# ViTAE-Transformer/LeMeViT

Measured on AMD Instinct MI355X. Metric: images/sec LeMeViT-Base 224^2 bf16 fwd+bwd, higher is better.
Workload: dtype bf16; 1 GPU; lemevit_base 224x224 bf16-autocast train step (fwd+bwd+AdamW), batch 128/GPU, drop_path 0.1, random-init weights; global_batch=128, parallelism=dp1, launch=eager, weight-gradient GEMMs on a side stream

## Files before the change

### include/lemevit_hip.h

```cpp
#ifndef LEMEVIT_HIP_H
#define LEMEVIT_HIP_H

#include <stddef.h>
#include <stdint.h>

#ifdef __cplusplus
extern "C" {
#endif

#define LMV_ABI_VERSION 14

enum { LMV_F32 = 0, LMV_BF16 = 1, LMV_U8 = 2  };
enum {
  LMV_OK = 0,
  LMV_ERR_SHAPE = -1,
  LMV_ERR_DTYPE = -2,
  LMV_ERR_WORKSPACE = -3,
  LMV_ERR_LAUNCH = -4
};

int lmv_abi_version(void);
const char* lmv_last_error(void);
int lmv_config_set(const char* key, int value);
int lmv_config_get(const char* key, int* value);
// ... 149 lines not shown
int lmv_row_scale(const void* x, const float* scale, void* y, int64_t rows, int C, int rows_per_sample, int dtype, void* stream);
typedef struct lmv_row_scale_segment {
  const void* x; const float* scale; void* y;
  int64_t rows; int rows_per_sample;
} lmv_row_scale_segment;
int lmv_row_scale_multi(const lmv_row_scale_segment* seg, int nseg, int C, int dtype, void* stream);
#define LMV_TRANSPOSE_MAX_SEGS 48
typedef struct { const void* src; void* dst; int32_t rows, cols; } lmv_transpose_seg;
int lmv_transpose_batch(const lmv_transpose_seg* segs, int nsegs, int dtype, void* stream);
int lmv_im2col3x3s2_nhwc(const void* x, void* patches, int B, int H, int W, int C, int KP, int dtype, void* stream);
int lmv_col2im3x3s2_nhwc(const void* dpatches, void* dx, int B, int H, int W, int C, int KP, int dtype, void* stream);
int lmv_conv3x3s2_fwd(const void* x, const void* wm, const float* bias, void* y, int B, int H, int W, int Cin, int Cout, int KP, int act, int dtype, void* stream);
size_t lmv_conv3x3s2_dw_workspace_bytes(int B, int H, int W, int Cin, int Cout, int KP, int dtype);
int lmv_conv3x3s2_dw(const void* dy, const void* x, float* dwm, float* dbias, int B, int H, int W, int Cin, int Cout, int KP, void* workspace, size_t workspace_bytes, int dtype,
                     void* stream);
enum { LMV_FOLD_CI_TAP = 0, LMV_FOLD_TAP_CI = 1 };
int lmv_conv_bn_fold(const float* w, const float* b, const float* gamma, const float* beta, const float* mean, const float* var, float eps, int Co, int Cin, int KP,
                     int layout, void* wm, float* bf, float* sc, int dtype, void* stream);
int lmv_conv_bn_fold_bwd(const float* dwm, const float* dbf, const float* w, const float* b, const float* gamma, const float* mean, const float* var, float eps, int Co,
                         int Cin, int KP, int layout, float* dW, float* db, float* dgamma, float* dbeta, void* stream);
int lmv_token_mean2_fwd(const void* x, int L, const void* c, int M, int C, int B, void* out, int dtype, void* stream);
int lmv_token_mean2_bwd(const void* g, void* dx, int L, void* dc, int M, int C, int B, int dtype, void* stream);
int lmv_token_mean2_affine_fwd(const void* x, int L, const void* c, int M, int C, int B, const float* xscale, const float* xshift, void* out, int dtype,
                               void* stream);
int lmv_adamw_flat(float* param, const float* grad, float* exp_avg, float* exp_avg_sq, const float* wd_mask, void* shadow_bf16,
                   int64_t n, float lr, float beta1, float beta2, float eps, float weight_decay, int step, const int* step_dev,
                   void* stream);
typedef struct { const float* ptr; int64_t n; } lmv_norm_seg;
#define LMV_GRAD_STAT_FLOATS 8
#define LMV_NORM_CHUNK 16384
// ... 206 lines not shown
```

### lemevit_amd/_lib.py

```python
from __future__ import annotations

import ctypes as C
import os

import torch

_HERE = os.path.dirname(os.path.abspath(__file__))
LIB_PATH = os.environ.get("LMV_LIB_PATH") or os.path.join(_HERE, "csrc", "liblemevit_hip.so")

LMV_F32, LMV_BF16, LMV_U8 = 0, 1, 2
ACT_NONE, ACT_GELU, ACT_GELU_GRAD, ACT_GELU_BWD = 0, 1, 2, 3
FOLD_CI_TAP, FOLD_TAP_CI = 0, 1
ABI_VERSION = 14
BLOCK_NO_JOIN, BLOCK_FUSED, BLOCK_DATA_ONLY = 1, 2, 4
GRAD_STAT_FLOATS, NORM_CHUNK, NORM_SKIP_NONFINITE = 8, 16384, 1
ADAMW_UNIT, ADAMW_MAX_GROUPS = 8, 256
ERASE_MAX_BOXES = 4
ERASE_CONST, ERASE_RAND, ERASE_PIXEL = 0, 1, 2
EVAL_MAX_PRED, METER_MAX_K = 16, 8
DENSE_MAX_CLASSES, DENSE_STATS_HEAD = 64, 6
DENSE_LABEL_I64, DENSE_LABEL_U8 = 0, 1
DENSE_AVG_VALID, DENSE_AVG_ALL, DENSE_AVG_WEIGHT = 0, 1, 2
DENSE_SLIDE_MAX_GRID = 64
RROI_MAX_LEVELS, RROI_MAX_SAMPLE_NUM, RROI_MAX_BINS, RROI_MAX_SAMPLES, RROI_MAX_EXTENT = 5, 4, 256, 1024, 65535
# ... 150 lines not shown
    "lmv_dca_core_fwd": (_I, [_P, _P, _P, _P, _P, _P, _I, _I, _I, _I, _P, _Z, _I, _P]),
    "lmv_cast": (_I, [_P, _I, _P, _I, _L, _P]),
    "lmv_im2col3x3s2_c3": (_I, [_P, _I, _P, _I, _I, _I, _I, _L, _L, _L, _L, _P]),
    "lmv_im2col3x3s2_nchw": (_I, [_P, _I, _P, _I, _I, _I, _I, _I, _I, _L, _L, _L, _L, _P]),
    "lmv_conv3x3s2_nchw_dx": (_I, [_P, _P, _P, _I, _I, _I, _I, _I, _I, _I, _L, _L, _L, _L, _I, _P]),
    "lmv_row_scale_multi": (_I, [_P, _I, _I, _I, _P]),
    "lmv_transpose_batch": (_I, [C.POINTER(TransposeSeg), _I, _I, _P]),
    "lmv_row_scale": (_I, [_P, _P, _P, _L, _I, _I, _I, _P]),
    "lmv_im2col3x3s2_nhwc": (_I, [_P, _P, _I, _I, _I, _I, _I, _I, _P]),
    "lmv_conv3x3s2_fwd": (_I, [_P, _P, _P, _P, _I, _I, _I, _I, _I, _I, _I, _I, _P]),
    "lmv_conv3x3s2_dw_workspace_bytes": (_Z, [_I, _I, _I, _I, _I, _I, _I]),
    "lmv_conv3x3s2_dw": (_I, [_P, _P, _P, _P, _I, _I, _I, _I, _I, _I, _P, _Z, _I, _P]),
    "lmv_conv_bn_fold": (_I, [_P, _P, _P, _P, _P, _P, _F, _I, _I, _I, _I, _P, _P, _P, _I, _P]),
    "lmv_conv_bn_fold_bwd": (_I, [_P, _P, _P, _P, _P, _P, _P, _F, _I, _I, _I, _I, _P, _P, _P, _P, _P]),
    "lmv_col2im3x3s2_nhwc": (_I, [_P, _P, _I, _I, _I, _I, _I, _I, _P]),
    "lmv_token_mean2_fwd": (_I, [_P, _I, _P, _I, _I, _I, _P, _I, _P]),
    "lmv_token_mean2_affine_fwd": (_I, [_P, _I, _P, _I, _I, _I, _P, _P, _P, _I, _P]),
    "lmv_token_mean2_bwd": (_I, [_P, _P, _I, _P, _I, _I, _I, _I, _P]),
    "lmv_adamw_flat": (_I, [_P, _P, _P, _P, _P, _P, _L, _F, _F, _F, _F, _F, _I, _P, _P]),
    "lmv_grad_norm_workspace_bytes": (_Z, [C.POINTER(NormSeg), _I]),
    "lmv_grad_norm": (_I, [C.POINTER(NormSeg), _I, _F, _I, _P, _P, _P, _Z, _P]),
    "lmv_adamw_flat_clip": (_I, [_P, _P, _P, _P, _P, _P, _L, _F, _F, _F, _F, _F, _I, _P, _P, _F, _P]),
    "lmv_adamw_flat_groups": (_I, [_P, _P, _P, _P, _P, _L, _P, _P, _I, _F, _F, _F, _I, _P, _P, _F, _P]),
    "lmv_ema_flat": (_I, [_P, _P, _L, _F, _P]),
    "lmv_mix_images": (_I, [_P, _I, _L, _L, _L, _L, _P, _I, _I, _I, _I, _I, _P, _P, _P, _P, _P]),
    "lmv_soft_ce": (_I, [_P, _I, _L, _I, _I, _P, _P, _F, _P, _I, _L, _P, _P, _P, _P]),
    "lmv_augment_images": (_I, [_P, _I, _L, _L, _L, _L, _P, _I, _I, _I, _I, _I, _P, _P, _P, _P, _I, _P, _P, _P, _P]),
    "lmv_eval_logits": (_I, [_P, _I, _L, _I, _I, _P, _I, _P, _P, _P, _I, _P]),
    "lmv_meter_add": (_I, [_P, _P, _P, _I, C.POINTER(C.c_int32), _I, _P, _L, _P]),
    "lmv_dense_loss_workspace_bytes": (_Z, [_I, _I, _L]),
# ... 96 lines not shown
```

### lemevit_amd/csrc/gemm.hip

```cpp
#include <stdlib.h>
#include <atomic>
#include <utility>
#include "common.h"

#include "gemm_tiles.h"

namespace {

template <typename T, bool ATR, bool BTR, bool SPLITK, int BK, bool DMA, typename CF, int MINW = 1, int NST = 2, bool LNP = false, bool CONV = false>
__global__ __launch_bounds__(CF::NTHR, MINW) void gemm_kernel(const GemmArgs g) {
  static_assert(!LNP || (!ATR && !BTR && !SPLITK), "the LayerNorm-folded epilogue belongs to the forward contraction");
  static_assert(!CONV || (DMA && ((!ATR && !BTR && !SPLITK) || (ATR && BTR && SPLITK))), "the implicit-GEMM convolution: the LDS-DMA forward and weight-gradient kernels");
  using RS = typename std::conditional<LNP, RowStat<CF::WM>, NoStat>::type;
  RS rstat;
  if constexpr (LNP) rstat.clear();
#ifdef LMV_GEMM_TIMING
  const bool tstamp = g.dbg && (threadIdx.x == 0) && (blockIdx.x == 0 || blockIdx.x == gridDim.x / 2);
  unsigned long long* const tdbg = g.dbg + (blockIdx.x == 0 ? 0 : 256);
  int tstn = 0;
#define GSTAMP() do { if (tstamp && tstn < 250) tdbg[tstn++] = __builtin_amdgcn_s_memtime(); } while (0)
#else
#define GSTAMP() do { } while (0)
#endif
  GSTAMP();
  constexpr int PANEL_BYTES = PANEL * BK * (int)sizeof(T);
  constexpr int BUF_BYTES = (CF::PA + CF::PB) * PANEL_BYTES;
  constexpr int WM = CF::WM;
// ... 15 lines not shown
    if (split >= g.nsplits || bid >= g.ntiles) return;
  } else {
    const int T_ = gridDim.x, xcd = blockIdx.x & 7, q = T_ >> 3, r = T_ & 7, len = q + (xcd < r ? 1 : 0);
    int idx = blockIdx.x >> 3;
    const int chunk = idx & ~127;
    if (chunk + 128 <= len) idx = chunk + ((idx & 31) << 2) + ((idx >> 5) & 3);
    bid = (xcd < r ? xcd * (q + 1) : r * (q + 1) + (xcd - r) * q) + idx;
  }
  const bool second = g.nprob > 1 && !g.concat && bid >= g.p[1].tile_begin;
  const int pi = second ? 1 : 0;
  Problem P;
#define LMV_SEL(f) P.f = second ? g.p[1].f : g.p[0].f
  LMV_SEL(a); LMV_SEL(b); LMV_SEL(bias); LMV_SEL(res); LMV_SEL(row_scale); LMV_SEL(aux); LMV_SEL(out); LMV_SEL(out_pre); LMV_SEL(bias_grad);
  LMV_SEL(M); LMV_SEL(Kred); LMV_SEL(rps); LMV_SEL(tiles_m); LMV_SEL(tile_begin);
#undef LMV_SEL
  bid -= P.tile_begin;
  const int tm = bid / g.tiles_n, tn = bid % g.tiles_n;
  const int m0 = tm * CF::BM, n0 = tn * CF::BN;
  const int M = P.M, N = g.N;
  const int kt0 = (P.Kred + BK - 1) / BK;
  const int kt_total = kt0 + ((SPLITK && g.concat) ? (g.p[1].Kred + BK - 1) / BK : 0);
  const int kt_beg = split * g.kt_per_split;
  const int kt_end = min(kt_total, kt_beg + g.kt_per_split);
  if (kt_beg >= kt_end) return;
  const T* const a0 = reinterpret_cast<const T*>(P.a); const T* const b0 = reinterpret_cast<const T*>(P.b);
  const T* const a1 = SPLITK ? reinterpret_cast<const T*>(g.p[1].a) : a0; const T* const b1 = SPLITK ? reinterpret_cast<const T*>(g.p[1].b) : b0;
  const int kred0 = P.Kred, kred1 = SPLITK ? g.p[1].Kred : P.Kred;
  auto src_of = [&](int kt, const T** a, const T** b, int* kred, int* k0) {
    const bool second = SPLITK && kt >= kt0;
    *a = second ? a1 : a0; *b = second ? b1 : b0;
// ... 7 lines not shown
#pragma unroll
    for (int j = 0; j < 4; ++j) acc[i][j] = f32x4_t{0.f, 0.f, 0.f, 0.f};
  }
  const int ra0 = wm * WM * 16, cb0 = wn * 64;
  const int pa = ra0 / PANEL, oa = ra0 % PANEL, pb = cb0 / PANEL, ob = cb0 % PANEL;
  const bool do_bsum = SPLITK && (P.bias_grad != nullptr) && tn == 0 && wn == 0;

  constexpr int REGION = NST * BUF_BYTES / CF::NW;
  constexpr bool EPI_EARLY = false;
  Epi<T, CF, SPLITK ? 4096 : REGION> epi;
  if constexpr (EPI_EARLY) epi.prefetch(P, g.act & 0xff, N, g.ldc, m0, n0, wm, wn, lane);

  int cur = 0;
  if constexpr (DMA) {
    static_assert(sizeof(T) == 2, "the direct-to-LDS path is bf16 only");
    auto issue = [&](unsigned char* buf, int kt) {
      const bf16_t *A16, *B16; int kred, k0;
      src_of(kt, &A16, &B16, &kred, &k0);
#pragma unroll
      for (int q = 0; q < CF::PA; ++q) {
        if constexpr (CONV && !SPLITK) panel_dma_conv<false, BK, CF::NW>(buf + q * PANEL_BYTES, g.cv, M, m0 + q * PANEL, k0, lane, wave);
        else panel_dma<ATR, BK, CF::NW>(buf + q * PANEL_BYTES, A16, g.lda, M, m0 + q * PANEL, k0, lane, wave);
      }
#pragma unroll
      for (int q = 0; q < CF::PB; ++q) {
        if constexpr (CONV && SPLITK) panel_dma_conv<true, BK, CF::NW>(buf + (CF::PA + q) * PANEL_BYTES, g.cv, N, n0 + q * PANEL, k0, lane, wave);
        else panel_dma<BTR, BK, CF::NW>(buf + (CF::PA + q) * PANEL_BYTES, B16, g.ldb, N, n0 + q * PANEL, k0, lane, wave);
      }
    };
    if constexpr (CF::NW >= 8 && CF::WM == 2 && NST == 2) {
      issue(smem, kt_beg);
      GSTAMP();
      __syncthreads();
      GSTAMP();
      for (int kt = kt_beg; kt < kt_end; ++kt) {
        if (kt + 1 < kt_end) issue(smem + (cur ^ 1) * BUF_BYTES, kt + 1);
        GSTAMP();
        const unsigned char* buf = smem + cur * BUF_BYTES;
        tile_mma<T, ATR, BTR, BK, SPLITK, WM, RS>(buf + pa * PANEL_BYTES, oa, buf + (CF::PA + pb) * PANEL_BYTES, ob, acc, accb, do_bsum, lane, &rstat);
        GSTAMP();
        __syncthreads();
// ... 69 lines not shown
      if (do_bsum && lane < 16) slab[(int64_t)M * g.ldc + m] = accb[ti][0];
    }
  } else {
    GSTAMP();
    if constexpr (LNP) {
      rstat.finish(P.Kred, g.ln_eps);
      epi.prefetch(P, LMV_ACT_NONE, N, g.ldc, m0, n0, wm, wn, lane);
      epi.template store<true>(smem, acc, P, g.act & 0xff, N, g.ldc, m0, n0, wm, wn, lane, wave, rstat.s, rstat.q);
    } else {
      if constexpr (!EPI_EARLY) epi.prefetch(P, g.act & 0xff, N, g.ldc, m0, n0, wm, wn, lane);
      GSTAMP();
#ifdef LMV_GEMM_TIMING
      auto est = [&]() { GSTAMP(); };
      epi.template store<false, decltype(est)>(smem, acc, P, g.act & 0xff, N, g.ldc, m0, n0, wm, wn, lane, wave, nullptr, nullptr, est);
#else
      epi.store(smem, acc, P, g.act & 0xff, N, g.ldc, m0, n0, wm, wn, lane, wave);
#endif
      GSTAMP();
    }
  }
}

template <int SL>
__global__ __launch_bounds__(256) void splitk_reduce_kernel(const float* __restrict__ ws, int nslabs, int64_t stride, float* __restrict__ out_w,
                                                           int64_t nw, float* __restrict__ out_b, int nb) {
  constexpr int EL = 256 / SL;
  __shared__ float4 red[SL > 1 ? 256 : 1];
  const int64_t n4 = (nw + (out_b ? nb : 0)) >> 2;
  const int e = threadIdx.x % EL, sl = threadIdx.x / EL;
  const int64_t i = (int64_t)blockIdx.x * EL + e;
  float4 a = make_float4(0.f, 0.f, 0.f, 0.f);
  if (i < n4) {
    const float* p = ws + i * 4;
#pragma unroll 8
    for (int s = sl; s < nslabs; s += SL) {
// ... 357 lines not shown
  return launch(&p, 1, Cout, KP, act, dtype, stream, MODE_FWD, nullptr, 0, nullptr, nullptr, &cv);
}
extern "C" size_t lmv_conv3x3s2_dw_workspace_bytes(int B, int H, int W, int Cin, int Cout, int KP, int dtype) {
  (void)Cin;
  lmv_linear_problem p{};
  p.a = p.w = p.out = (void*)16; p.rows = (int64_t)B * ((H + 1) / 2) * ((W + 1) / 2);
  return lmv_linear_dw_workspace_bytes(&p, 1, Cout, KP, dtype);
}
extern "C" int lmv_conv3x3s2_dw(const void* dy, const void* x, float* dwm, float* dbias, int B, int H, int W, int Cin, int Cout, int KP, void* workspace, size_t workspace_bytes, int dtype,
                                void* stream) {
  ConvGeo cv;
  LMV_TRY(conv_geo(&cv, x, B, H, W, Cin, Cout, KP, dtype));
  lmv_linear_problem p{};
  p.a = dy; p.w = x; p.out = dwm; p.bias_grad = dbias; p.rows = (int64_t)B * cv.HoWo;
  return launch(&p, 1, Cout, KP, LMV_ACT_NONE, dtype, stream, MODE_DW, workspace, workspace_bytes, nullptr, nullptr, &cv);
}

extern "C" int lmv_reduce_batch(const lmv_reduce_seg* segs, int nsegs, void* stream) {
  if (nsegs <= 0) return LMV_OK;
  if (!segs) LMV_FAIL(LMV_ERR_SHAPE, "reduce_batch: segs is NULL");
  hipStream_t st = (hipStream_t)stream;
  for (int s0 = 0; s0 < nsegs; s0 += LMV_REDUCE_MAX_SEGS) {
    ReduceBatch rb{};
    rb.n = nsegs - s0 < LMV_REDUCE_MAX_SEGS ? nsegs - s0 : LMV_REDUCE_MAX_SEGS;
    int blocks = 0;
    for (int i = 0; i < rb.n; ++i) {
      const lmv_reduce_seg& q = segs[s0 + i];
      if (!q.ws || !q.out_w || q.nslabs <= 0 || q.nw <= 0 || (q.nw % 4) || (q.out_b && (q.nb % 4)) || !lmv_aligned16(q.ws) || !lmv_aligned16(q.out_w) ||
          !lmv_aligned16(q.out_b) || (q.slab_stride % 4) || (q.kind != LMV_REDUCE_SLABS && q.kind != LMV_REDUCE_ROWS))
        LMV_FAIL(LMV_ERR_SHAPE, "reduce_batch: bad segment %d", s0 + i);
// ... 22 lines not shown
```

### lemevit_amd/csrc/gemm_tiles.h

```cpp
#pragma once
#include <utility>
#include "common.h"

namespace {

constexpr int PANEL = 128;

template <int NWM_, int NWN_, int WM_>
struct Cfg {
  static constexpr int NWM = NWM_, NWN = NWN_, WM = WM_;
  static constexpr int NW = NWM * NWN, NTHR = NW * 64;
  static constexpr int BM = NWM * WM * 16, BN = NWN * 64;
  static constexpr int PA = BM / PANEL, PB = BN / PANEL;
};
using C128 = Cfg<2, 2, 4>;
using C128w8 = Cfg<4, 2, 2>;

struct Problem {
  const void* a; const void* b; const float* bias; const void* res; const float* row_scale; const void* aux;
  void* out; void* out_pre; float* bias_grad;
  int M;
  int Kred;
  int rps;
  int tiles_m;
  int tile_begin;
  int pad_;
};
struct ReduceSegDev { const float* ws; float* out_w; float* out_b; int64_t stride, nw; int nslabs, nb, sl, blk0, kind, mode; };
#define LMV_CV_SHIFT 41
struct ConvGeo {
  int on, H, W, Cin, Ho, Wo, HoWo, pad_;
  unsigned long long m_cin, m_wo, m_howo;
  const void* x;
};
struct GemmArgs {
  Problem p[2];
  int nprob, N, lda, ldb, ldc, act, tiles_n, kt_per_split;
  ConvGeo cv;
  int ntiles, nsplits, concat;
  float ln_eps;
#ifdef LMV_GEMM_TIMING
  unsigned long long* dbg;
#endif
  float* ws;
  int64_t slab_stride;
  int slab_base[2];
};

template <int ROWB> __device__ __forceinline__ int swz_n(int row) { return ROWB == 64 ? ((-(row >> 2)) & 3) : ((row >> 1) & 7); }
// ... 35 lines not shown
      const int row = c / CPR, kc = c % CPR;
      off = row * ROWB + ((kc ^ swz_n<ROWB>(row)) << 4);
    } else {
      constexpr int CPR = PANEL / EPC;
      const int r = c / CPR, cc = c % CPR;
      if (sizeof(T) == 2) off = r * 256 + ((((cc >> 1) ^ swz_t(r))) << 5) + ((cc & 1) << 4);
      else off = r * 512 + (cc << 4);
    }
    *reinterpret_cast<uint4*>(s + off) = regs[i];
  }
}

typedef __attribute__((address_space(3))) void* lds_vp;
typedef const __attribute__((address_space(1))) void* glb_vp;

template <bool TR, int BK, int NW>
__device__ __forceinline__ void panel_dma(unsigned char* panel, const bf16_t* __restrict__ base, int64_t ld, int dim, int tile0, int k0,
                                          int lane, int wave) {
  constexpr int NSEG = PANEL * BK * 2 / 1024;
  static_assert(NSEG % NW == 0, "segments must divide over the waves");
#pragma unroll
  for (int i = 0; i < NSEG / NW; ++i) {
    const int sg = wave + i * NW;
    const bf16_t* src;
    if (!TR) {
      constexpr int ROWB = BK * 2, CPR = ROWB / 16, RPS = 1024 / ROWB;
      const int r = sg * RPS + lane / CPR, p = lane % CPR, kc = p ^ swz_n<ROWB>(r);
      src = base + (int64_t)min(tile0 + r, dim - 1) * ld + k0 + kc * 8;
    } else {
      const int r = sg * 4 + (lane >> 4), p16 = lane & 15, c16 = ((((p16 >> 1) ^ swz_t(r))) << 1) | (p16 & 1);
      src = base + (int64_t)(k0 + r) * ld + min(tile0 + c16 * 8, dim - 8);
    }
    __builtin_amdgcn_global_load_lds((glb_vp)src, (lds_vp)(panel + sg * 1024), 16, 0, 0);
  }
// ... 15 lines not shown
  static_assert(NSEG % NW == 0, "segments must divide over the waves");
#pragma unroll
  for (int i = 0; i < NSEG / NW; ++i) {
    const int sg = wave + i * NW;
    const bf16_t* src;
    if (!TR) {
      constexpr int ROWB = BK * 2, CPR = ROWB / 16, RPS = 1024 / ROWB;
      const int r = sg * RPS + lane / CPR, p = lane % CPR, kc = p ^ swz_n<ROWB>(r);
      src = cv_src(cv, min(tile0 + r, dim - 1), k0 + kc * 8);
    } else {
      const int r = sg * 4 + (lane >> 4), p16 = lane & 15, c16 = ((((p16 >> 1) ^ swz_t(r))) << 1) | (p16 & 1);
      src = cv_src(cv, k0 + r, min(tile0 + c16 * 8, dim - 8));
    }
    __builtin_amdgcn_global_load_lds((glb_vp)src, (lds_vp)(panel + sg * 1024), 16, 0, 0);
  }
}

template <bool TR, int BK>
__device__ __forceinline__ bf16x8_t frag_bf16(const unsigned char* s, int base, int lane, int hh) {
  if (!TR) {
    constexpr int ROWB = BK * 2;
    const int row = base + (lane & 15), kc = hh * 4 + (lane >> 4);
    return *reinterpret_cast<const bf16x8_t*>(s + row * ROWB + ((kc ^ swz_n<ROWB>(row)) << 4));
  } else {
    const int g = lane >> 4, i = lane & 15, rr = i >> 2, q = i & 3;
    const int r1 = hh * 32 + g * 8 + rr, r2 = r1 + 4, ch = base >> 4;
    typedef __attribute__((address_space(3))) bf16x4_t* lds4_t;
    bf16x4_t lo = __builtin_amdgcn_ds_read_tr16_b64_v4bf16((lds4_t)(s + r1 * 256 + ((ch ^ swz_t(r1)) << 5) + q * 8));
    bf16x4_t hi = __builtin_amdgcn_ds_read_tr16_b64_v4bf16((lds4_t)(s + r2 * 256 + ((ch ^ swz_t(r2)) << 5) + q * 8));
    return __builtin_shufflevector(lo, hi, 0, 1, 2, 3, 4, 5, 6, 7);
// ... 233 lines not shown
            const int m = min(m0 + wm * (CF::WM * 16) + p * RPP + r, P.M - 1);
            rs[p][i] = P.row_scale[m / P.rps];
          }
      }
    }
    if constexpr (HOIST_BIAS) {
#pragma unroll
      for (int tj = 0; tj < 4; ++tj) b4[tj] = bias_at(P, N, nw0 + tj * 16 + (lane >> 4) * 4);
    }
  }
  static __device__ __forceinline__ float4 bias_at(const Problem& P, int N, int n) {
    return (P.bias && n < N) ? *reinterpret_cast<const float4*>(P.bias + n) : make_float4(0.f, 0.f, 0.f, 0.f);
  }

  struct NoStamp { __device__ __forceinline__ void operator()() const {} };
  template <bool LN = false, typename ST = NoStamp>
  __device__ __forceinline__ void store(unsigned char* smem, const f32x4_t (&acc)[CF::WM][4], const Problem& P, int act, int N, int64_t ldc,
                                        int m0, int n0, int wm, int wn, int lane, int wave, const float* ln_mean = nullptr, const float* ln_rstd = nullptr,
                                        ST stamp = ST{}) const {
    float* sT = reinterpret_cast<float*>(smem + wave * REGION_BYTES);
    T* outp = reinterpret_cast<T*>(P.out);
    T* prep = reinterpret_cast<T*>(P.out_pre);
    const int nw0 = n0 + wn * 64;
#pragma unroll
    for (int p = 0; p < NPASS; ++p) {
      __builtin_amdgcn_wave_barrier();
#pragma unroll
      for (int tj = 0; tj < 4; ++tj) {
        float4 b;
        if constexpr (HOIST_BIAS) b = b4[tj]; else b = bias_at(P, N, nw0 + tj * 16 + (lane >> 4) * 4);
        float4 cs = make_float4(0.f, 0.f, 0.f, 0.f);
        if constexpr (LN) {
          const int n = nw0 + tj * 16 + (lane >> 4) * 4;
          if (n < N) cs = *reinterpret_cast<const float4*>(reinterpret_cast<const float*>(P.aux) + n);
// ... 13 lines not shown
      asm volatile("s_waitcnt lgkmcnt(0)" ::: "memory");
      __builtin_amdgcn_wave_barrier();
      stamp();
#pragma unroll
      for (int i = 0; i < NITER; ++i) {
        const int c = lane + i * 64, r = c / CPR, oc = c % CPR;
        const int m = m0 + wm * (CF::WM * 16) + p * RPP + r, n = nw0 + oc * EPC;
        if (m >= P.M || n >= N) continue;
        float v[EPC];
#pragma unroll
        for (int e = 0; e < EPC; e += 4) {
          const int c4 = (oc * EPC + e) >> 2;
          const float4 t = *reinterpret_cast<const float4*>(sT + r * 64 + ((c4 ^ (r & 7)) << 2));
          v[e] = t.x; v[e + 1] = t.y; v[e + 2] = t.z; v[e + 3] = t.w;
        }
        const int64_t o = (int64_t)m * ldc + n;
        if (prep) *reinterpret_cast<uint4*>(prep + o) = f_to_chunk<T>(v);
        if (act == LMV_ACT_GELU) {
#pragma unroll
          for (int e = 0; e < EPC; ++e) v[e] = act_gelu<T>(v[e]);
        } else if (act == LMV_ACT_GELU_GRAD) {
          float u[EPC];
          chunk_to_f<T>(pf[p][i], u);
#pragma unroll
          for (int e = 0; e < EPC; ++e) v[e] *= act_gelu_grad<T>(u[e]);
        }
        if (P.row_scale) {
          float sc;
          if constexpr (HOIST_BIAS) sc = rs[p][i]; else sc = P.row_scale[m / P.rps];
#pragma unroll
          for (int e = 0; e < EPC; ++e) v[e] *= sc;
// ... 17 lines not shown
```

### lemevit_amd/model.py

```python
from __future__ import annotations

import math
import operator
import os
import threading
import weakref
from collections import OrderedDict
from typing import Dict, List, Optional, Sequence, Tuple

import torch
import torch.nn as nn
import torch.nn.functional as F

from . import ops
from .blocks import ATTN_BWD, ATTN_FWD, BLOCK_LN_EPS, PARAM_NAMES, attention_state, block_backward, block_forward
from .ops import Prob

Tensor = torch.Tensor


def _cfg(url: str = "", **kwargs) -> dict:
    return dict(url=url, num_classes=1000, input_size=(3, 224, 224), pool_size=None, crop_pct=0.9, interpolation="bicubic",
                fixed_input_size=True, mean=(0.485, 0.456, 0.406), std=(0.229, 0.224, 0.225),
                first_conv="patch_embed.proj", classifier="head", **kwargs)
# ... 153 lines not shown
            dwm = torch.zeros(Co, KP, device=g.device, dtype=torch.float32)
            dbf = torch.zeros(Co, device=g.device, dtype=torch.float32)
            if ctx.form == "implicit":
                ops.conv3x3s2_dw(g, gathered, dwm, dbf)
            else:
                ops.linear_dw([Prob(g, gathered, dwm, bias_grad=dbf)], Co, KP)
            if folded:
                weight, bias, gamma, mean, var = sv[-5:]
                grads = list(ops.conv_bn_fold_bwd(dwm, dbf, weight, bias, gamma, mean, var, eps, layout, [bool(n) for n in need]))
            else:
                dw = dwm[:, :9 * Ci]
                dw = dw.reshape(wshape) if image else dw.reshape(Co, 3, 3, Ci).permute(0, 3, 1, 2)
                grads[:2] = (dw.to(wdt) if need[0] else None), (dbf.to(bdt) if need[1] else None)
        if need_x and image:
            dx = ops.conv3x3s2_nchw_dx(g, Wm, like=sv[0])
        elif need_x:
            dp = torch.empty(g.shape[0], KP, device=g.device, dtype=g.dtype)
            ops.linear_dx([Prob(g, Wm, dp)], Co, KP)
            dx = ops.col2im3x3s2_nhwc(dp, B, H, W, Ci).permute(0, 3, 1, 2).to(xdt)
        return (dx, grads[0], grads[1], None, grads[2], grads[3], None, None, None, None, None)


def _conv3x3s2(x: Tensor, weight: Tensor, bias: Optional[Tensor], cd: torch.dtype, bn: Optional[tuple] = None, gelu: bool = False, infer: bool = False) -> Tensor:
    if (infer or (gelu and bn is None)) and torch.is_grad_enabled() and any(t is not None and t.requires_grad for t in (x, weight, bias)):
        raise NotImplementedError("lemevit_amd: the inference fold and the fused GELU epilogue on a plain operand have no backward")
    gamma, beta, mean, var, eps = (None, None, None, None, None) if bn is None else bn
    return _Conv3x3s2Fn.apply(x, weight, bias, cd, gamma, beta, mean, var, eps, gelu, infer)


def _is_conv3x3s2p1(m: nn.Module) -> bool:
    return (isinstance(m, nn.Conv2d) and m.kernel_size == (3, 3) and m.stride == (2, 2) and m.padding == (1, 1) and m.dilation == (1, 1) and m.groups == 1
            and m.padding_mode == "zeros")


def _is_conv3x3s2(m: nn.Module, x: Tensor) -> bool:
    return (_is_conv3x3s2p1(m) and m.in_channels % 8 == 0 and m.out_channels % 8 == 0 and x.is_cuda
            and x.dtype in (torch.float32, torch.bfloat16) and m.weight.dtype in (torch.float32, torch.bfloat16))


_CONV_IMPLICIT = os.environ.get("LMV_CONV_IMPLICIT", "1") != "0"


_FROZEN_BN = os.environ.get("LMV_FROZEN_BN", "1") != "0"


def _bn_frozen(m: Optional[nn.Module]) -> bool:
    return (_FROZEN_BN and isinstance(m, nn.BatchNorm2d) and not m.training and m.track_running_stats and m.running_mean is not None and m.running_var is not None
            and m.affine and all(t.dtype == torch.float32 for t in (m.weight, m.bias, m.running_mean, m.running_var)))


def _conv_bn_pairs(m: nn.Module, bn: Optional[nn.Module], x: Tensor, cd: torch.dtype) -> bool:
    return (_bn_frozen(bn) and cd in (torch.float32, torch.bfloat16) and x.is_cuda and (_is_stem_conv1(m, x) or _is_conv3x3s2(m, x)) and m.weight.dtype == torch.float32
            and (m.bias is None or m.bias.dtype == torch.float32) and m.weight.is_contiguous() and bn.num_features == m.out_channels)


# ... 1502 lines not shown
```

### lemevit_amd/ops.py

```python
from __future__ import annotations

import ctypes as C
import math
from typing import List, Optional, Sequence, Tuple

import torch

from . import _lib
from ._lib import ACT_GELU, ACT_GELU_BWD, ACT_GELU_GRAD, ACT_NONE, FOLD_CI_TAP, FOLD_TAP_CI, AttnDesc, LinearProblem, LnSegment, check, lib

Tensor = torch.Tensor
HEAD_DIM = 32


def dtype_code(t: Tensor) -> int:
    if t.dtype == torch.float32:
        return _lib.LMV_F32
    if t.dtype == torch.bfloat16:
        return _lib.LMV_BF16
    raise TypeError(f"lemevit_amd: unsupported dtype {t.dtype} (float32 and bfloat16 only)")


_raw_stream = getattr(torch._C, "_cuda_getCurrentRawStream", None)

# ... 501 lines not shown
def conv_bn_fold_bwd(dwm: Tensor, dbf: Tensor, weight: Tensor, bias: Optional[Tensor], gamma: Tensor, mean: Tensor, var: Tensor, eps: float, layout: int,
                     want: Sequence[bool] = (True, True, True, True)):
    Co, Cin = weight.shape[0], weight.shape[1]
    if dwm.shape[0] != Co or dbf.numel() != Co:
        raise ValueError(f"conv_bn_fold_bwd: dwm {tuple(dwm.shape)} / dbf {tuple(dbf.shape)} do not match the weight {tuple(weight.shape)}")
    new = lambda w, shape: torch.empty(shape, device=weight.device, dtype=torch.float32) if w else None
    dW, db, dg, dbe = new(want[0], weight.shape), new(want[1], (Co,)), new(want[2], (Co,)), new(want[3], (Co,))
    check(lib.lmv_conv_bn_fold_bwd(_f32(dwm), _f32(dbf), _f32(weight), _f32(bias), _f32(gamma), _f32(mean), _f32(var), eps, Co, Cin, dwm.shape[1], layout,
                                   _ptr(dW), _ptr(db), _ptr(dg), _ptr(dbe), _stream()), "lmv_conv_bn_fold_bwd")
    return dW, db, dg, dbe


def col2im3x3s2_nhwc(dpatches: Tensor, B: int, H: int, W: int, C_: int) -> Tensor:
    dx = torch.empty((B, H, W, C_), device=dpatches.device, dtype=dpatches.dtype)
    check(lib.lmv_col2im3x3s2_nhwc(_ptr(dpatches), _ptr(dx), B, H, W, C_, dpatches.shape[1], dtype_code(dpatches), _stream()), "lmv_col2im3x3s2_nhwc")
    return dx


def token_mean2_fwd(x: Tensor, c: Optional[Tensor]) -> Tensor:
    B, L, C_ = x.shape
    out = torch.empty((B, C_), device=x.device, dtype=x.dtype)
    check(lib.lmv_token_mean2_fwd(_ptr(x), L, _ptr(c), 0 if c is None else c.shape[1], C_, B, _ptr(out), dtype_code(x), _stream()), "lmv_token_mean2_fwd")
    return out


def token_mean2_affine_fwd(x: Tensor, c: Optional[Tensor], xscale: Tensor, xshift: Tensor) -> Tensor:
    B, L, C_ = x.shape
    if xscale.dtype != torch.float32 or xshift.dtype != torch.float32 or xscale.numel() != C_ or xshift.numel() != C_:
        raise TypeError("token_mean2_affine_fwd: xscale / xshift must be float32 [C]")
    out = torch.empty((B, C_), device=x.device, dtype=x.dtype)
# ... 1204 lines not shown
```

Measured before the change: 4262 images/sec.

## Add implicit-GEMM data-gradient kernel for 3x3 stride-2 convs with parity-class decomposition

Replaces the conv3x3s2 input-gradient path (linear_dx into a materialized patch matrix, then col2im) with a single implicit-GEMM kernel. Output pixels are split into four stride-parity classes, each gathering only its contributing taps from dy via LDS-DMA, and results are written straight to NHWC dx. A cached transposed weight operand is built per weight version. This removes the large dpatches buffer and the col2im scatter pass, at the cost of gather address arithmetic, zero-page loads at borders, and a new code path with shape limits.

```diff
diff --git a/include/lemevit_hip.h b/include/lemevit_hip.h
--- a/include/lemevit_hip.h
+++ b/include/lemevit_hip.h
@@ -187,6 +187,9 @@
 size_t lmv_conv3x3s2_dw_workspace_bytes(int B, int H, int W, int Cin, int Cout, int KP, int dtype);
 int lmv_conv3x3s2_dw(const void* dy, const void* x, float* dwm, float* dbias, int B, int H, int W, int Cin, int Cout, int KP, void* workspace, size_t workspace_bytes, int dtype,
                      void* stream);
+int lmv_conv3x3s2_dx_supported(int B, int H, int W, int Cin, int Cout, int dtype);
+int lmv_conv3x3s2_dx_operand(const void* wm, void* wt, int Cin, int Cout, int KP, int dtype, void* stream);
+int lmv_conv3x3s2_dx(const void* dy, const void* wt, void* dx, int B, int H, int W, int Cin, int Cout, int dtype, void* stream);
 enum { LMV_FOLD_CI_TAP = 0, LMV_FOLD_TAP_CI = 1 };
 int lmv_conv_bn_fold(const float* w, const float* b, const float* gamma, const float* beta, const float* mean, const float* var, float eps, int Co, int Cin, int KP,
                      int layout, void* wm, float* bf, float* sc, int dtype, void* stream);
diff --git a/lemevit_amd/_lib.py b/lemevit_amd/_lib.py
--- a/lemevit_amd/_lib.py
+++ b/lemevit_amd/_lib.py
@@ -188,6 +188,9 @@
     "lmv_conv_bn_fold": (_I, [_P, _P, _P, _P, _P, _P, _F, _I, _I, _I, _I, _P, _P, _P, _I, _P]),
     "lmv_conv_bn_fold_bwd": (_I, [_P, _P, _P, _P, _P, _P, _P, _F, _I, _I, _I, _I, _P, _P, _P, _P, _P]),
     "lmv_col2im3x3s2_nhwc": (_I, [_P, _P, _I, _I, _I, _I, _I, _I, _P]),
+    "lmv_conv3x3s2_dx_supported": (_I, [_I, _I, _I, _I, _I, _I]),
+    "lmv_conv3x3s2_dx_operand": (_I, [_P, _P, _I, _I, _I, _I, _P]),
+    "lmv_conv3x3s2_dx": (_I, [_P, _P, _P, _I, _I, _I, _I, _I, _I, _P]),
     "lmv_token_mean2_fwd": (_I, [_P, _I, _P, _I, _I, _I, _P, _I, _P]),
     "lmv_token_mean2_affine_fwd": (_I, [_P, _I, _P, _I, _I, _I, _P, _P, _P, _I, _P]),
     "lmv_token_mean2_bwd": (_I, [_P, _P, _I, _P, _I, _I, _I, _I, _P]),
diff --git a/lemevit_amd/csrc/gemm.hip b/lemevit_amd/csrc/gemm.hip
--- a/lemevit_amd/csrc/gemm.hip
+++ b/lemevit_amd/csrc/gemm.hip
@@ -7,10 +7,10 @@
 
 namespace {
 
-template <typename T, bool ATR, bool BTR, bool SPLITK, int BK, bool DMA, typename CF, int MINW = 1, int NST = 2, bool LNP = false, bool CONV = false>
-__global__ __launch_bounds__(CF::NTHR, MINW) void gemm_kernel(const GemmArgs g) {
+template <typename T, bool ATR, bool BTR, bool SPLITK, int BK, bool DMA, typename CF, int NST, bool LNP, int CONV, typename DX>
+__device__ __forceinline__ void gemm_body(const GemmArgs& g, const DX& d) {
   static_assert(!LNP || (!ATR && !BTR && !SPLITK), "the LayerNorm-folded epilogue belongs to the forward contraction");
-  static_assert(!CONV || (DMA && ((!ATR && !BTR && !SPLITK) || (ATR && BTR && SPLITK))), "the implicit-GEMM convolution: the LDS-DMA forward and weight-gradient kernels");
+  static_assert(!CONV || (DMA && ((!ATR && !BTR && !SPLITK) || (CONV == 1 && ATR && BTR && SPLITK))), "the implicit-GEMM convolution: the LDS-DMA forward and weight-gradient kernels");
   using RS = typename std::conditional<LNP, RowStat<CF::WM>, NoStat>::type;
   RS rstat;
   if constexpr (LNP) rstat.clear();
@@ -56,6 +56,17 @@
   LMV_SEL(a); LMV_SEL(b); LMV_SEL(bias); LMV_SEL(res); LMV_SEL(row_scale); LMV_SEL(aux); LMV_SEL(out); LMV_SEL(out_pre); LMV_SEL(bias_grad);
   LMV_SEL(M); LMV_SEL(Kred); LMV_SEL(rps); LMV_SEL(tiles_m); LMV_SEL(tile_begin);
 #undef LMV_SEL
+  ConvDxClass dc{};
+  if constexpr (CONV == 2) {
+    const int r_ = bid / g.tiles_n, cls = r_ & 3;
+#define LMV_SELD(f) dc.f = cls == 0 ? d.c[0].f : cls == 1 ? d.c[1].f : cls == 2 ? d.c[2].f : d.c[3].f
+    LMV_SELD(M); LMV_SELD(Kred); LMV_SELD(boff); LMV_SELD(Wc); LMV_SELD(HcWc); LMV_SELD(py); LMV_SELD(px); LMV_SELD(m_wc); LMV_SELD(m_hcwc);
+#undef LMV_SELD
+    P.M = dc.M; P.Kred = dc.Kred;
+    P.b = reinterpret_cast<const T*>(P.b) + dc.boff;
+    if ((r_ >> 2) * CF::BM >= dc.M) return;
+    bid = (r_ >> 2) * g.tiles_n + (bid - r_ * g.tiles_n);
+  }
   bid -= P.tile_begin;
   const int tm = bid / g.tiles_n, tn = bid % g.tiles_n;
   const int m0 = tm * CF::BM, n0 = tn * CF::BN;
@@ -93,17 +104,22 @@
   int cur = 0;
   if constexpr (DMA) {
     static_assert(sizeof(T) == 2, "the direct-to-LDS path is bf16 only");
+    static_assert(CONV != 2 || (CF::PA == 1 && BK == 32), "the data-gradient gather: one A panel, k-tiles inside one tap");
+    DxRow dxrow[CONV == 2 ? PANEL * BK * 2 / 1024 / CF::NW : 1];
+    if constexpr (CONV == 2) convdx_rows<BK, CF::NW>(dxrow, d, dc, M, m0, lane, wave);
     auto issue = [&](unsigned char* buf, int kt) {
       const bf16_t *A16, *B16; int kred, k0;
       src_of(kt, &A16, &B16, &kred, &k0);
 #pragma unroll
       for (int q = 0; q < CF::PA; ++q) {
-        if constexpr (CONV && !SPLITK) panel_dma_conv<false, BK, CF::NW>(buf + q * PANEL_BYTES, g.cv, M, m0 + q * PANEL, k0, lane, wave);
+        if constexpr (CONV == 1 && !SPLITK) panel_dma_conv<false, BK, CF::NW>(buf + q * PANEL_BYTES, g.cv, M, m0 + q * PANEL, k0, lane, wave);
+        else if constexpr (CONV == 2) panel_dma_convdx<BK, CF::NW>(buf + q * PANEL_BYTES, d, dc, dxrow, k0, wave);
         else panel_dma<ATR, BK, CF::NW>(buf + q * PANEL_BYTES, A16, g.lda, M, m0 + q * PANEL, k0, lane, wave);
       }
 #pragma unroll
       for (int q = 0; q < CF::PB; ++q) {
-        if constexpr (CONV && SPLITK) panel_dma_conv<true, BK, CF::NW>(buf + (CF::PA + q) * PANEL_BYTES, g.cv, N, n0 + q * PANEL, k0, lane, wave);
+        if constexpr (CONV == 1 && SPLITK) panel_dma_conv<true, BK, CF::NW>(buf + (CF::PA + q) * PANEL_BYTES, g.cv, N, n0 + q * PANEL, k0, lane, wave);
+        else if constexpr (CONV == 2 && CF::BN < PANEL) panel_dma<BTR, BK, CF::NW, CF::BN>(buf + (CF::PA + q) * PANEL_BYTES, B16, g.ldb, N, n0 + q * PANEL, k0, lane, wave);
         else panel_dma<BTR, BK, CF::NW>(buf + (CF::PA + q) * PANEL_BYTES, B16, g.ldb, N, n0 + q * PANEL, k0, lane, wave);
       }
     };
@@ -203,11 +219,25 @@
       auto est = [&]() { GSTAMP(); };
       epi.template store<false, decltype(est)>(smem, acc, P, g.act & 0xff, N, g.ldc, m0, n0, wm, wn, lane, wave, nullptr, nullptr, est);
 #else
-      epi.store(smem, acc, P, g.act & 0xff, N, g.ldc, m0, n0, wm, wn, lane, wave);
+      if constexpr (CONV == 2) {
+        auto rowmap = [&](int m) { return cv_row_dx(d, dc, m); };
+        epi.template store<false, typename decltype(epi)::NoStamp, decltype(rowmap)>(smem, acc, P, LMV_ACT_NONE, N, g.ldc, m0, n0, wm, wn, lane, wave, nullptr, nullptr, {}, rowmap);
+      } else {
+        epi.store(smem, acc, P, g.act & 0xff, N, g.ldc, m0, n0, wm, wn, lane, wave);
+      }
 #endif
       GSTAMP();
     }
   }
+}
+
+template <typename T, bool ATR, bool BTR, bool SPLITK, int BK, bool DMA, typename CF, int MINW = 1, int NST = 2, bool LNP = false, bool CONV = false>
+__global__ __launch_bounds__(CF::NTHR, MINW) void gemm_kernel(const GemmArgs g) {
+  gemm_body<T, ATR, BTR, SPLITK, BK, DMA, CF, NST, LNP, CONV ? 1 : 0>(g, NoDx{});
+}
+template <typename CF>
+__global__ __launch_bounds__(CF::NTHR, 4) void conv_dx_kernel(const GemmArgs g, const ConvDxArgs d) {
+  gemm_body<bf16_t, false, false, false, 32, true, CF, 2, false, 2>(g, d);
 }
 
 template <int SL>
@@ -595,6 +625,72 @@
   lmv_linear_problem p{};
   p.a = dy; p.w = x; p.out = dwm; p.bias_grad = dbias; p.rows = (int64_t)B * cv.HoWo;
   return launch(&p, 1, Cout, KP, LMV_ACT_NONE, dtype, stream, MODE_DW, workspace, workspace_bytes, nullptr, nullptr, &cv);
+}
+
+namespace {
+__global__ __launch_bounds__(256) void conv_dx_operand_kernel(const unsigned short* __restrict__ wm, unsigned short* __restrict__ wt, int Cin, int Cout, int KP) {
+  const int K9 = 9 * Cout;
+  const int idx = blockIdx.x * 256 + threadIdx.x;
+  if (idx >= Cin * K9) return;
+  const int ci = idx / K9, c = idx - ci * K9, q = c / Cout, co = c - q * Cout;
+  int ky, kx;
+  if (q == 0) { ky = 1; kx = 1; }
+  else if (q < 3) { ky = 1; kx = 2 * (q - 1); }
+  else if (q < 5) { ky = 2 * (q - 3); kx = 1; }
+  else { ky = 2 * ((q - 5) >> 1); kx = 2 * ((q - 5) & 1); }
+  wt[idx] = wm[(int64_t)co * KP + (ky * 3 + kx) * Cin + ci];
+}
+
+bool conv_dx_shape_ok(int B, int H, int W, int Cin, int Cout) {
+  if (B <= 0 || H <= 0 || W <= 0 || Cin <= 0 || Cout <= 0 || (Cin % 8) || (Cout % 32) || Cout >= (1 << 11)) return false;
+  const int64_t hc = (H + 1) / 2, wc = (W + 1) / 2;
+  return hc * wc < (1 << 19) && (int64_t)B * hc * wc < (1 << 22) && (int64_t)B * H * W * Cin < (1LL << 31) && (int64_t)B * hc * wc * Cout < (1LL << 31);
+}
+}
+extern "C" int lmv_conv3x3s2_dx_supported(int B, int H, int W, int Cin, int Cout, int dtype) { return dtype == LMV_BF16 && conv_dx_shape_ok(B, H, W, Cin, Cout) ? 1 : 0; }
+extern "C" int lmv_conv3x3s2_dx_operand(const void* wm, void* wt, int Cin, int Cout, int KP, int dtype, void* stream) {
+  if (dtype != LMV_BF16) LMV_FAIL(LMV_ERR_DTYPE, "conv3x3s2_dx_operand: bf16 only");
+  if (Cin <= 0 || Cout <= 0 || (Cin % 8) || (Cout % 8) || KP < 9 * Cin || (int64_t)Cin * 9 * Cout >= (1LL << 31) || (int64_t)Cout * KP >= (1LL << 31))
+    LMV_FAIL(LMV_ERR_SHAPE, "conv3x3s2_dx_operand: Cin, Cout multiples of 8, KP >= 9 Cin");
+  if (!wm || !wt || !lmv_aligned16(wm) || !lmv_aligned16(wt)) LMV_FAIL(LMV_ERR_SHAPE, "conv3x3s2_dx_operand: null / misaligned operand");
+  const int n = Cin * 9 * Cout;
+  hipLaunchKernelGGL(conv_dx_operand_kernel, dim3((n + 255) / 256), dim3(256), 0, (hipStream_t)stream, reinterpret_cast<const unsigned short*>(wm),
+                     reinterpret_cast<unsigned short*>(wt), Cin, Cout, KP);
+  LMV_CHECK_LAUNCH("conv3x3s2_dx_operand");
+  return LMV_OK;
+}
+extern "C" int lmv_conv3x3s2_dx(const void* dy, const void* wt, void* dx, int B, int H, int W, int Cin, int Cout, int dtype, void* stream) {
+  if (dtype != LMV_BF16) LMV_FAIL(LMV_ERR_DTYPE, "conv3x3s2_dx: bf16 only (fp32: lmv_linear_dx + lmv_col2im3x3s2_nhwc)");
+  if (!conv_dx_shape_ok(B, H, W, Cin, Cout))
+    LMV_FAIL(LMV_ERR_SHAPE, "conv3x3s2_dx: Cin %% 8, Cout %% 32, Cout < 2048, B Ho Wo < 2^22, Ho Wo < 2^19, maps < 2^31 elements (B=%d H=%d W=%d Cin=%d Cout=%d)", B, H, W, Cin, Cout);
+  if (!dy || !wt || !dx || !lmv_aligned16(dy) || !lmv_aligned16(wt) || !lmv_aligned16(dx)) LMV_FAIL(LMV_ERR_SHAPE, "conv3x3s2_dx: null / misaligned operand");
+  const bool narrow = Cin <= 64;
+  const int bn = narrow ? C128n64::BN : C128::BN;
+  auto magic = [](unsigned d) { return ((1ull << LMV_CV_SHIFT) + d - 1) / d; };
+  ConvDxArgs d{};
+  d.H = H; d.W = W; d.Ho = (H + 1) / 2; d.Wo = (W + 1) / 2; d.Cout = Cout; d.dy = dy; d.m_cout = magic((unsigned)Cout);
+  GemmArgs g{};
+  g.nprob = 1; g.N = Cin; g.lda = Cout; g.ldb = 9 * Cout; g.ldc = Cin; g.act = LMV_ACT_NONE; g.tiles_n = (Cin + bn - 1) / bn; g.kt_per_split = 4 * Cout / 32; g.nsplits = 1;
+  int off = 0;
+  for (int cls = 0; cls < 4; ++cls) {
+    const int py = cls >> 1, px = cls & 1, taps = (1 + py) * (1 + px);
+    const int hc = (H - py + 1) / 2, wc = (W - px + 1) / 2;
+    ConvDxClass& c = d.c[cls];
+    c.M = B * hc * wc; c.Kred = taps * Cout; c.boff = off; c.Wc = wc; c.HcWc = hc * wc; c.py = py; c.px = px;
+    c.m_wc = magic((unsigned)(wc > 0 ? wc : 1)); c.m_hcwc = magic((unsigned)(hc * wc > 0 ? hc * wc : 1));
+    off += taps * Cout;
+  }
+  Problem& P = g.p[0];
+  P.a = dy; P.b = wt; P.out = dx; P.M = d.c[0].M; P.Kred = Cout; P.rps = 1; P.tiles_m = (P.M + 127) / 128; P.tile_begin = 0;
+  const int total = 4 * P.tiles_m * g.tiles_n;
+  g.ntiles = total;
+  const double px_ = (double)B * H * W, rows = (double)B * d.Ho * d.Wo;
+  LmvTimedLaunch timed(stream, 2.0 * 9.0 * Cout * Cin * rows, 2.0 * (rows * Cout + px_ * Cin + 9.0 * Cout * Cin), LMV_TK_GEMM_DX);
+  constexpr int lds = 2 * 2 * PANEL * 32 * 2;
+  if (narrow) hipLaunchKernelGGL(conv_dx_kernel<C128n64>, dim3(total), dim3(C128n64::NTHR), lds, (hipStream_t)stream, g, d);
+  else hipLaunchKernelGGL(conv_dx_kernel<C128>, dim3(total), dim3(C128::NTHR), lds, (hipStream_t)stream, g, d);
+  LMV_CHECK_LAUNCH("conv3x3s2_dx");
+  return LMV_OK;
 }
 
 extern "C" int lmv_reduce_batch(const lmv_reduce_seg* segs, int nsegs, void* stream) {
diff --git a/lemevit_amd/csrc/gemm_tiles.h b/lemevit_amd/csrc/gemm_tiles.h
--- a/lemevit_amd/csrc/gemm_tiles.h
+++ b/lemevit_amd/csrc/gemm_tiles.h
@@ -11,9 +11,10 @@
   static constexpr int NWM = NWM_, NWN = NWN_, WM = WM_;
   static constexpr int NW = NWM * NWN, NTHR = NW * 64;
   static constexpr int BM = NWM * WM * 16, BN = NWN * 64;
-  static constexpr int PA = BM / PANEL, PB = BN / PANEL;
+  static constexpr int PA = BM / PANEL, PB = (BN + PANEL - 1) / PANEL;
 };
 using C128 = Cfg<2, 2, 4>;
+using C128n64 = Cfg<4, 1, 2>;
 using C128w8 = Cfg<4, 2, 2>;
 
 struct Problem {
@@ -33,6 +34,14 @@
   unsigned long long m_cin, m_wo, m_howo;
   const void* x;
 };
+struct ConvDxClass { int M, Kred, boff, Wc, HcWc, py, px, pad_; unsigned long long m_wc, m_hcwc; };
+struct ConvDxArgs {
+  ConvDxClass c[4];
+  int H, W, Ho, Wo, Cout, pad_;
+  unsigned long long m_cout;
+  const void* dy;
+};
+struct NoDx {};
 struct GemmArgs {
   Problem p[2];
   int nprob, N, lda, ldb, ldc, act, tiles_n, kt_per_split;
@@ -98,10 +107,11 @@
 typedef __attribute__((address_space(3))) void* lds_vp;
 typedef const __attribute__((address_space(1))) void* glb_vp;
 
-template <bool TR, int BK, int NW>
+template <bool TR, int BK, int NW, int NROWS = PANEL>
 __device__ __forceinline__ void panel_dma(unsigned char* panel, const bf16_t* __restrict__ base, int64_t ld, int dim, int tile0, int k0,
                                           int lane, int wave) {
-  constexpr int NSEG = PANEL * BK * 2 / 1024;
+  static_assert(NROWS == PANEL || !TR, "a partial panel is a partial set of rows");
+  constexpr int NSEG = NROWS * BK * 2 / 1024;
   static_assert(NSEG % NW == 0, "segments must divide over the waves");
 #pragma unroll
   for (int i = 0; i < NSEG / NW; ++i) {
@@ -147,6 +157,36 @@
     }
     __builtin_amdgcn_global_load_lds((glb_vp)src, (lds_vp)(panel + sg * 1024), 16, 0, 0);
   }
+}
+
+struct DxRow { int off; unsigned ok; };
+template <int BK, int NW>
+__device__ __forceinline__ void convdx_rows(DxRow (&rw)[PANEL * BK * 2 / 1024 / NW], const ConvDxArgs& d, const ConvDxClass& c, int dim, int tile0, int lane, int wave) {
+  constexpr int ROWB = BK * 2, CPR = ROWB / 16, RPS = 1024 / ROWB;
+#pragma unroll
+  for (int q = 0; q < PANEL * BK * 2 / 1024 / NW; ++q) {
+    const int sg = wave + q * NW, r = sg * RPS + lane / CPR, p = lane % CPR, kc = p ^ swz_n<ROWB>(r);
+    const unsigned n = (unsigned)min(tile0 + r, dim - 1);
+    const unsigned b = cv_div(n, c.m_hcwc), rem = n - b * (unsigned)c.HcWc, i = cv_div(rem, c.m_wc), j = rem - i * (unsigned)c.Wc;
+    rw[q].off = (((int)b * d.Ho + (int)i) * d.Wo + (int)j) * d.Cout + kc * 8;
+    rw[q].ok = (i + 1u < (unsigned)d.Ho ? 1u : 0u) | (j + 1u < (unsigned)d.Wo ? 2u : 0u);
+  }
+}
+template <int BK, int NW>
+__device__ __forceinline__ void panel_dma_convdx(unsigned char* panel, const ConvDxArgs& d, const ConvDxClass& c, const DxRow (&rw)[PANEL * BK * 2 / 1024 / NW], int k0, int wave) {
+  const unsigned t = cv_div((unsigned)k0, d.m_cout), ty = c.px ? t >> 1 : t, tx = c.px ? t & 1u : 0u;
+  const int doy = c.py - (int)ty, dox = c.px - (int)tx;
+  const int tapoff = (doy * d.Wo + dox) * d.Cout + (k0 - (int)t * d.Cout);
+  const unsigned need = (unsigned)doy | ((unsigned)dox << 1);
+#pragma unroll
+  for (int q = 0; q < PANEL * BK * 2 / 1024 / NW; ++q) {
+    const bf16_t* src = (rw[q].ok & need) == need ? reinterpret_cast<const bf16_t*>(d.dy) + ((unsigned)rw[q].off + (unsigned)tapoff) : reinterpret_cast<const bf16_t*>(lmv_zero_page);
+    __builtin_amdgcn_global_load_lds((glb_vp)src, (lds_vp)(panel + (wave + q * NW) * 1024), 16, 0, 0);
+  }
+}
+__device__ __forceinline__ int64_t cv_row_dx(const ConvDxArgs& d, const ConvDxClass& c, int n) {
+  const unsigned b = cv_div((unsigned)n, c.m_hcwc), rem = (unsigned)n - b * (unsigned)c.HcWc, i = cv_div(rem, c.m_wc), j = rem - i * (unsigned)c.Wc;
+  return (int64_t)((int)b * d.H + 2 * (int)i + c.py) * d.W + 2 * (int)j + c.px;
 }
 
 template <bool TR, int BK>
@@ -410,10 +450,11 @@
   }
 
   struct NoStamp { __device__ __forceinline__ void operator()() const {} };
-  template <bool LN = false, typename ST = NoStamp>
+  struct RowIdent { __device__ __forceinline__ int64_t operator()(int m) const { return m; } };
+  template <bool LN = false, typename ST = NoStamp, typename RM = RowIdent>
   __device__ __forceinline__ void store(unsigned char* smem, const f32x4_t (&acc)[CF::WM][4], const Problem& P, int act, int N, int64_t ldc,
                                         int m0, int n0, int wm, int wn, int lane, int wave, const float* ln_mean = nullptr, const float* ln_rstd = nullptr,
-                                        ST stamp = ST{}) const {
+                                        ST stamp = ST{}, RM rowmap = RM{}) const {
     float* sT = reinterpret_cast<float*>(smem + wave * REGION_BYTES);
     T* outp = reinterpret_cast<T*>(P.out);
     T* prep = reinterpret_cast<T*>(P.out_pre);
@@ -457,7 +498,7 @@
           const float4 t = *reinterpret_cast<const float4*>(sT + r * 64 + ((c4 ^ (r & 7)) << 2));
           v[e] = t.x; v[e + 1] = t.y; v[e + 2] = t.z; v[e + 3] = t.w;
         }
-        const int64_t o = (int64_t)m * ldc + n;
+        const int64_t o = rowmap(m) * ldc + n;
         if (prep) *reinterpret_cast<uint4*>(prep + o) = f_to_chunk<T>(v);
         if (act == LMV_ACT_GELU) {
 #pragma unroll
diff --git a/lemevit_amd/model.py b/lemevit_amd/model.py
--- a/lemevit_amd/model.py
+++ b/lemevit_amd/model.py
@@ -191,6 +191,10 @@
                 grads[:2] = (dw.to(wdt) if need[0] else None), (dbf.to(bdt) if need[1] else None)
         if need_x and image:
             dx = ops.conv3x3s2_nchw_dx(g, Wm, like=sv[0])
+        elif need_x and _CONV_DX and ops.conv3x3s2_dx_ok(g, B, H, W, Ci, Co):
+            Wt = derived(Wm, ("conv_dx",), (Wm,), lambda: ops.conv3x3s2_dx_operand(Wm, Ci))
+            dx = ops.conv3x3s2_dx(g, Wt, B, H, W).permute(0, 3, 1, 2)
+            dx = dx if dx.dtype == xdt else dx.to(xdt)
         elif need_x:
             dp = torch.empty(g.shape[0], KP, device=g.device, dtype=g.dtype)
             ops.linear_dx([Prob(g, Wm, dp)], Co, KP)
@@ -216,6 +220,9 @@
 
 
 _CONV_IMPLICIT = os.environ.get("LMV_CONV_IMPLICIT", "1") != "0"
+
+
+_CONV_DX = os.environ.get("LMV_CONV_DX", "1") != "0"
 
 
 _FROZEN_BN = os.environ.get("LMV_FROZEN_BN", "1") != "0"
diff --git a/lemevit_amd/ops.py b/lemevit_amd/ops.py
--- a/lemevit_amd/ops.py
+++ b/lemevit_amd/ops.py
@@ -539,6 +539,32 @@
 def col2im3x3s2_nhwc(dpatches: Tensor, B: int, H: int, W: int, C_: int) -> Tensor:
     dx = torch.empty((B, H, W, C_), device=dpatches.device, dtype=dpatches.dtype)
     check(lib.lmv_col2im3x3s2_nhwc(_ptr(dpatches), _ptr(dx), B, H, W, C_, dpatches.shape[1], dtype_code(dpatches), _stream()), "lmv_col2im3x3s2_nhwc")
+    return dx
+
+
+def conv3x3s2_dx_ok(dy: Tensor, B: int, H: int, W: int, C_: int, Cout: int) -> bool:
+    Ho, Wo = (H + 1) // 2, (W + 1) // 2
+    return (dy.is_cuda and dy.dtype == torch.bfloat16 and dy.is_contiguous() and dy.data_ptr() % 16 == 0 and min(B, H, W, C_, Cout) > 0 and C_ % 8 == 0 and Cout % 32 == 0
+            and Cout < (1 << 11) and Ho * Wo < (1 << 19) and B * Ho * Wo < (1 << 22) and B * H * W * C_ < (1 << 31) and B * Ho * Wo * Cout < (1 << 31))
+
+
+def conv3x3s2_dx_operand(wm: Tensor, C_: int) -> Tensor:
+    Co, KP = wm.shape
+    if wm.dtype != torch.bfloat16 or not wm.is_contiguous():
+        raise TypeError("conv3x3s2_dx_operand: takes the contiguous bf16 operand [Cout, KP]")
+    wt = torch.empty((C_, 9 * Co), device=wm.device, dtype=wm.dtype)
+    check(lib.lmv_conv3x3s2_dx_operand(_ptr(wm), _ptr(wt), C_, Co, KP, dtype_code(wm), _stream()), "lmv_conv3x3s2_dx_operand")
+    return wt
+
+
+def conv3x3s2_dx(dy: Tensor, wt: Tensor, B: int, H: int, W: int, out: Optional[Tensor] = None) -> Tensor:
+    C_, Co = wt.shape[0], wt.shape[1] // 9
+    if dy.dtype != wt.dtype or dy.shape != (B * ((H + 1) // 2) * ((W + 1) // 2), Co) or not dy.is_contiguous() or not wt.is_contiguous():
+        raise ValueError(f"conv3x3s2_dx: dy {tuple(dy.shape)} {dy.dtype} does not match wt {tuple(wt.shape)} {wt.dtype} and the map {(B, H, W, C_)}")
+    dx = torch.empty((B, H, W, C_), device=dy.device, dtype=dy.dtype) if out is None else out
+    if dx.shape != (B, H, W, C_) or dx.dtype != dy.dtype or not dx.is_contiguous():
+        raise ValueError("conv3x3s2_dx: out must be a contiguous [B, H, W, Cin] tensor of dy's dtype")
+    check(lib.lmv_conv3x3s2_dx(_ptr(dy), _ptr(wt), _ptr(dx), B, H, W, C_, Co, dtype_code(dy), _stream()), "lmv_conv3x3s2_dx")
     return dx
 
 
```

New measurement: 4289 images/sec (median of 4 runs). No clear change (+0.6%).
